# shanmo/OrcVIO

Measured on AMD Instinct MI355X. Metric: EKF updates/sec, 30 clones x 400 feats, higher is better.
Workload: dtype f64

## Files before the change

orcvio_amd/csrc/capi_handle.inc:

```

static double reg_lower_gamma(double a, double x) {
    if (x <= 0.0) return 0.0;
    const double lg = std::lgamma(a);
    if (x < a + 1.0) {
        double term = 1.0 / a, sum = term, ap = a;
        for (int i = 0; i < 200000; ++i) {
            ap += 1.0;
            term *= x / ap;
            sum += term;
            if (std::fabs(term) < std::fabs(sum) * 1e-17) break;
        }
        return sum * std::exp(a * std::log(x) - x - lg);
    }
    const double tiny = 1e-300;
    double b = x + 1.0 - a, c = 1.0 / tiny, d = 1.0 / b, h = d;
    for (int i = 1; i < 200000; ++i) {
        const double an = -(double)i * ((double)i - a);
        b += 2.0;
        d = an * d + b;
        if (std::fabs(d) < tiny) d = tiny;
        c = b + an / c;
        if (std::fabs(c) < tiny) c = tiny;
        d = 1.0 / d;
        const double del = d * c;
// ... 134 lines not shown
    size_t o = 0;
    for (int i = 0; i < n; ++i) {
        if (c[i].bytes == 0 || !c[i].dst) continue;
        HIPCHK(hipMemcpyAsync(h->h_fetch + o, c[i].src, c[i].bytes, hipMemcpyDeviceToHost, s));
        o += (c[i].bytes + 63) & ~(size_t)63;
    }
    HIPCHK(hipStreamSynchronize(s));
    o = 0;
    for (int i = 0; i < n; ++i) {
        if (c[i].bytes == 0 || !c[i].dst) continue;
        std::memcpy(c[i].dst, h->h_fetch + o, c[i].bytes);
        o += (c[i].bytes + 63) & ~(size_t)63;
    }
    return ORCVIO_OK;
}

static int launch_ingest(orcvio_msckf_handle* h, hipStream_t s, const void* src_dev, void* dst, size_t bytes, bool kernel = true,
                         int* zero = nullptr, unsigned zero_mask = 0u) {
    if (bytes == 0) return ORCVIO_OK;
    if (!kernel) {
        HIPCHK(hipMemcpyAsync(dst, src_dev, bytes, hipMemcpyHostToDevice, s));
        if (zero)
            for (int i = 0; i < 32; ++i)
                if (zero_mask >> i & 1u) HIPCHK(hipMemsetAsync(zero + i, 0, sizeof(int), s));
        return ORCVIO_OK;
    }
    const size_t n16 = (bytes + 15) / 16;
    int grid = (int)((n16 + 255) / 256);
    if (grid > 4 * h->n_cus) grid = 4 * h->n_cus;
    if (grid < 1) grid = 1;
    hipLaunchKernelGGL(k_ingest, dim3(grid), dim3(256), 0, s, reinterpret_cast<const u32x4*>(src_dev), reinterpret_cast<u32x4*>(dst), n16, zero, zero_mask);
    HIPCHK(hipGetLastError());
    return ORCVIO_OK;
}
static bool obj_ingest_kernel() {
    static const bool v = [] { const char* e = dbg_getenv("ORCVIO_OBJ_INGEST"); return e ? atoi(e) != 0 : true; }();
    return v;
}
static bool obj_publish_kernel() {
    static const bool v = [] { const char* e = dbg_getenv("ORCVIO_OBJ_PUBLISH"); return e ? atoi(e) != 0 : false; }();
    return v;
}
static void free_all(orcvio_msckf_handle* h) {
    (void)hipDeviceSynchronize();
    void* ptrs[] = {h->d_in, h->d_outs,
                    h->d_chi2, h->d_Hs, h->d_Gpart, h->d_Ab, h->d_A, h->d_RP,
                    h->d_DinvP, h->d_U, h->d_M, h->d_RM, h->d_DinvM, h->d_Z, h->d_La, h->d_DinvA,
                    h->d_W, h->d_Y, h->d_KG, h->d_Gobj, h->d_RF, h->d_DinvF, h->d_Yobj, h->d_objH,
                    h->d_obj_gamma, h->d_obj_i, h->d_obj_accept, h->d_T3, h->d_Xobs, h->d_S,
                    h->d_Pres, h->d_Ptmp, h->d_Sres, h->d_Stmp, h->d_covT, h->d_covmap, h->d_skip, h->d_tri_valid, h->d_tri_flags, h->d_tri_init, h->d_tri_sol, h->d_tri_cost, h->d_sync, h->d_la_rdy, h->d_U2, h->d_M2, h->d_RM2, h->d_DinvM2, h->d_Z2, h->d_outs2, h->d_chain_words, h->d_obj_done,
                    h->d_ekf_i, h->d_ekf_d, h->d_ekf_E, h->d_Gekf, h->d_ekf_gamma, h->d_ekf_accept, h->d_slam, h->d_dense, h->d_Rf, h->d_new, h->d_aug, h->d_split};
    for (void* p : ptrs)
        if (p) (void)hipFree(p);
    if (h->h_stage) (void)hipHostFree(h->h_stage);
    if (h->h_obj_stage) (void)hipHostFree(h->h_obj_stage);
    if (h->h_lm) (void)hipHostFree(h->h_lm);
    if (h->d_lm) (void)hipFree(h->d_lm);
    if (h->h_stage2) (void)hipHostFree(h->h_stage2);
    if (h->h_tri) (void)hipHostFree(h->h_tri);
    if (h->d_tri_words) (void)hipFree(h->d_tri_words);
    if (h->d_in2) (void)hipFree(h->d_in2);
    if (h->d_step_words) (void)hipFree(h->d_step_words);
    if (h->h_evt) (void)hipHostFree(h->h_evt);
    if (h->d_evt) (void)hipFree(h->d_evt);
    for (double* q : {h->d_Hthin, h->d_Vthin, h->d_uthin}) if (q) (void)hipFree(q);
    if (h->d_obj_in) (void)hipFree(h->d_obj_in);
// ... 338 lines not shown
```

orcvio_amd/csrc/capi_io.inc:

```

static int compute_optional(orcvio_msckf_handle* h, bool want_thin_or_K, bool want_K, bool want_G) {
    if (h->last_update_thin) { g_last_error = "H_thin / K / G are derived from the square-root path's factors: not available behind an update that took the direct form of a thin stack (ask for them in the update call itself)"; return ORCVIO_ERR_INVALID; }
    const int NA = h->NA, NAP = h->NAP, n = h->n, kf = h->kf - h->tail, NP = h->NP, ldz = h->ldz;
    hipStream_t s = h->stream;
    const PriorFactor pf = prior_factor(h);
    const long sLi = pf.sLi, sLj = pf.sLj;
    const double* La_P = pf.base + 15 * sLi;
    { const int ra = assemble_deferred(h, s); if (ra != ORCVIO_OK) return ra; }
    if (want_thin_or_K) {
        HIPCHK(hipMemcpyAsync(h->d_La, h->d_A, sizeof(double) * (size_t)NAP * NAP, hipMemcpyDeviceToDevice, s));
        hipLaunchKernelGGL(k_potrf, dim3(1), dim3(1024), 0, s, h->d_La, NA + 1, NAP, 0.0, h->d_DinvA, h->d_info + 4, 1e-11);
        HIPCHK(hipGetLastError());
    }
    if (want_G) {
        int rc = launch_trsm(h, s, h->d_RM, h->d_DinvM, kf, h->d_U, 1, NP, NA, nullptr, 0, h->d_W, NP);
        if (rc == ORCVIO_OK) rc = launch_gemm(s, h->d_Z, 1, ldz, h->d_W, NP, 1, n, NA, kf, 1.0, 0.0, 0, h->d_KG, NP, 1);
        if (rc != ORCVIO_OK) return rc;
    }
    if (want_K) {
        int rc = launch_gemm(s, La_P, sLj, sLi, h->d_La, NAP, 1, kf, NA, NA, 1.0, 0.0, 0, h->d_Y, NP, 1);
        if (rc == ORCVIO_OK) rc = launch_trsm(h, s, h->d_RM, h->d_DinvM, kf, h->d_Y, NP, 1, NA, nullptr, 0, h->d_W, NP);
        if (rc == ORCVIO_OK) rc = launch_gemm(s, h->d_Z, 1, ldz, h->d_W, NP, 1, n, NA, kf, 1.0, 0.0, 0, h->d_Y, NP, 1);
        if (rc != ORCVIO_OK) return rc;
    }
    HIPCHK(hipStreamSynchronize(s));
    return ORCVIO_OK;
}

static int download_enqueue(orcvio_msckf_handle* h, hipStream_t sd, bool with_P) {
    const size_t bytes = with_P ? h->oo_Pout + sizeof(double) * (size_t)h->n * h->n : h->outs_small;
    HIPCHK(hipMemcpyAsync(h->h_stage + h->in_cap + h->out_shift, h->d_outs, bytes, hipMemcpyDeviceToHost, sd));
    h->dl_pending = true; h->dl_with_P = with_P; h->dl_stream = sd;
    return ORCVIO_OK;
}

static int rerun_forked(orcvio_msckf_handle* h, hipStream_t s, bool want_P) {
    UpdateCall c;
    c.retry_forked = true;
    int rr = run_update_impl(h, s, c);
    if (rr == ORCVIO_OK) rr = download_enqueue(h, s ? s : h->stream, want_P);
    return rr;
}

static int download_impl(orcvio_msckf_handle* h, orcvio_msckf_result* res, bool retried) {
    if (!h || !res || !h->ran) { g_last_error = "download: no finished update"; return ORCVIO_ERR_INVALID; }
    HIPCHK(hipSetDevice(h->device));
    const int n = h->n, NA = h->NA, NAP = h->NAP, NP = h->NP, F = h->F;
    const bool want_P = res->P_out != nullptr;
    if (!(h->dl_pending && (h->dl_with_P || !want_P))) {
        hipStream_t sd = h->last_stream ? h->last_stream : h->stream;
        if (h->dl_pending) HIPCHK(hipStreamSynchronize(h->dl_stream));
        HIPCHK(hipStreamSynchronize(h->side));
        const int rq = download_enqueue(h, sd, want_P);
        if (rq != ORCVIO_OK) return rq;
    }
    HIPCHK(hipStreamSynchronize(h->dl_stream));
    h->dl_pending = false;
    if (h->last_sharded) {
        const int rl = ipc_check_lost(h, "orcvio_msckf_download");
        if (rl != ORCVIO_OK) return rl;
    }
    const char* so = h->h_stage + h->in_cap;
    const double* dx = reinterpret_cast<const double*>(so + h->oo_dx);
    const double* gam = reinterpret_cast<const double*>(so + h->oo_gamma);
    const int* acc = reinterpret_cast<const int*>(so + h->oo_accept);
    if (res->dx) std::memcpy(res->dx, dx, sizeof(double) * n);
    if (res->P_out) std::memcpy(res->P_out, so + h->oo_Pout, sizeof(double) * (size_t)n * n);
    if (res->accept && F > 0) std::memcpy(res->accept, acc, sizeof(int) * F);
    if (res->gamma && F > 0) std::memcpy(res->gamma, gam, sizeof(double) * F);
    int info[16] = {0};
    std::memcpy(info, so, sizeof(int) * 16);
// ... 40 lines not shown
        if (res->G) {
            std::vector<double> Gd((size_t)n * NP);
            HIPCHK(hipMemcpy(Gd.data(), h->d_KG, sizeof(double) * Gd.size(), hipMemcpyDeviceToHost));
            std::memset(res->G, 0, sizeof(double) * (size_t)n * n);
            for (int i = 0; i < n; ++i)
                for (int c = 0; c < NA; ++c) res->G[(size_t)i * n + 15 + c] = Gd[(size_t)i * NP + c];
        }
        if (res->K) {
            std::vector<double> Kd((size_t)n * NP);
            HIPCHK(hipMemcpy(Kd.data(), h->d_Y, sizeof(double) * Kd.size(), hipMemcpyDeviceToHost));
            for (int i = 0; i < n; ++i)
                for (int c = 0; c < NA; ++c) res->K[(size_t)i * NA + c] = Kd[(size_t)i * NP + c];
        }
    }
    return ORCVIO_OK;
}
int32_t orcvio_msckf_download(orcvio_msckf_handle* h, orcvio_msckf_result* res) { return download_impl(h, res, false); }

static int launch_triangulate(orcvio_msckf_handle* h, const orcvio_triangulation_config* cfg, bool have_init, bool mark_skip, hipStream_t s,
                              bool io, bool with_mode);
static inline void tri_consume(orcvio_msckf_handle* h, UpdateCall& c) {
    if (!h->tri_armed) return;
    h->tri_armed = false;
    c.tri = true;
    h->skip_active = true; h->tri_live = true;
    h->tri_refuse_empty = h->F > 0 && h->ekf_F == 0 && h->dense_rows == 0 && h->new_F == 0 && !c.info_also;
    if (h->tri_refuse_empty) c.info_also = h->d_tri_words;
}
static unsigned long long io_signature(const orcvio_msckf_handle* h, hipStream_t s, bool want_P, bool commit, const UpdateCall& c, bool finpub = false) {
    unsigned long long sig = launch_signature(h, s, h->h_stage_dev, (long)(0x100 | (want_P ? 1 : 0) | (commit ? 2 : 0) | (finpub ? 4 : 0)), c);
    auto mix = [&](unsigned long long v) { sig = (sig ^ v) * 1099511628211ull; };
    mix((unsigned long long)upload_bytes(h)); mix((unsigned long long)h->io_poses); mix((unsigned long long)(size_t)h->d_Stmp); mix((unsigned long long)(size_t)h->d_Pres);
    mix(h->factor_opt); mix((unsigned long long)h->outs_small); mix((unsigned long long)(size_t)h->d_Ptmp); mix(h->finpub_opt);
    mix(c.tri); mix(h->tri_live);
    if (c.tri) {
        const orcvio_triangulation_config& t = h->tri_cfg;
        const double d[6] = {t.translation_threshold, t.huber_epsilon, t.estimation_precision, t.initial_damping, t.cost_threshold, t.init_final_dist_threshold};
        for (double v : d) { unsigned long long bits; std::memcpy(&bits, &v, 8); mix(bits); }
        mix((unsigned long long)t.outer_loop_max_iteration); mix((unsigned long long)t.inner_loop_max_iteration);
        mix(h->tri_with_mode); mix((unsigned long long)(size_t)h->h_tri_dev); mix((unsigned long long)(size_t)c.info_also);
    }
    return sig;
}

static int step_words(orcvio_msckf_handle* h) {
    if (h->d_step_words) return ORCVIO_OK;
    HIPCHK(hipMalloc(&h->d_step_words, 256));
    HIPCHK(hipMemset(h->d_step_words, 0, 256));
    return ORCVIO_OK;
}

static inline bool finpub_active(const orcvio_msckf_handle* h, const UpdateCall& c) {
    return h->finpub_opt && !h->objects_mode && h->n_nui == 0 && !finish_fused_active(h, c);
}
static int io_enqueue(orcvio_msckf_handle* h, hipStream_t s, bool want_P, bool commit, UpdateCall& c, bool allow_finpub = false) {
    const int mode = commit ? (h->factor_opt && h->n_nui == 0 ? 2 : 1) : 0;
    const SolveOut so = solve_out(h);
    c.fin_pub = allow_finpub && finpub_active(h, c) && !want_P;
    if (c.fin_pub) c.pub = finish_pub_args(h, so, mode, c.info_also);
    h->last_finpub_commit = c.fin_pub && commit;
    int rc = ORCVIO_OK;
    if (!c.already_ingested) rc = launch_ingest(h, s, h->h_stage_dev, h->d_in, early_ingest() || (h->tri_live && !c.tri) ? h->io_poses : upload_bytes(h));
    if (rc == ORCVIO_OK && c.tri) rc = launch_triangulate(h, &h->tri_cfg, false, true, s, true, h->tri_with_mode);
    if (rc == ORCVIO_OK) rc = enqueue_update(h, s, c);
    if (rc != ORCVIO_OK || c.fin_pub) return rc;
    return launch_epilogue(s, epilogue_args(h, so, 0, want_P, mode, nullptr, c.info_also, c.info_keep));
}

static int io_wait(orcvio_msckf_handle* h, hipStream_t s, unsigned long long expected_pub) {
    const unsigned long long expected = expected_pub ? expected_pub : h->pub_enqueued;
    const auto t0 = std::chrono::steady_clock::now();
    unsigned spins = 0;
    bool late = false;
    while (__atomic_load_n(h->h_flag, __ATOMIC_ACQUIRE) < expected) {
        _mm_pause();
        if ((++spins & 4095u) == 0 &&
            std::chrono::duration<double>(std::chrono::steady_clock::now() - t0).count() > h->io_spin_seconds) { late = true; break; }
    }
    if (late) {
        HIPCHK(hipStreamSynchronize(s));
        const unsigned long long now = __atomic_load_n(h->h_flag, __ATOMIC_ACQUIRE);
        if (now < expected) {
            h->pub_enqueued = now;
            g_last_error = "io_update: the results were not published";
            return ORCVIO_ERR_TIMEOUT;
        }
    }
    return ORCVIO_OK;
}

struct FeatureView { int n, F, NA; size_t oo_dx, oo_gamma, oo_accept; const int* row_ptr; int discard_large_update; };
static inline FeatureView feature_view(const orcvio_msckf_handle* h) {
    return FeatureView{h->n, h->F, h->NA, h->oo_dx, h->oo_gamma, h->oo_accept, h->h_row_ptr.data(), h->flags.discard_large_update};
}
static int feature_outcome_view(orcvio_msckf_handle* h, const FeatureView& v, const char* so, int32_t* stats);
// ... 103 lines not shown
    return ORCVIO_OK;
}

int32_t orcvio_msckf_io_begin(orcvio_msckf_handle* h, const orcvio_msckf_flags* flags, int32_t n_clones, int32_t n_features,
                              int32_t n_observations, int32_t with_P, orcvio_msckf_io* io) {
    if (!h || !flags || !io) { g_last_error = "io_begin: null argument"; return ORCVIO_ERR_INVALID; }
    if (with_P < 0 || with_P > 2) { g_last_error = "io_begin: with_P is 0, 1 or 2"; return ORCVIO_ERR_INVALID; }
    const int rc = upload_begin(h, flags, n_clones, n_features, n_observations, with_P == 1, true, "orcvio_msckf_io_begin", with_P == 2);
    if (rc != ORCVIO_OK) return rc;
    char* st = h->h_stage;
    io->n = h->n;
    io->poses = reinterpret_cast<double*>(st + h->io_poses);
    io->obs_ptr = reinterpret_cast<int32_t*>(st + h->io_optr);
    io->p_w = reinterpret_cast<double*>(st + h->io_pw);
    io->obs_clone = reinterpret_cast<int32_t*>(st + h->io_oclone);
    io->obs_z = reinterpret_cast<double*>(st + h->io_z);
    io->obs_zvel = h->io_zvel != h->io_z ? reinterpret_cast<double*>(st + h->io_zvel) : nullptr;
    io->P = with_P == 1 ? reinterpret_cast<double*>(st + h->io_P) : nullptr;
    const char* so = st + h->in_cap;
    io->dx = reinterpret_cast<const double*>(so + h->oo_dx);
    io->gamma = reinterpret_cast<const double*>(so + h->oo_gamma);
    io->accept = reinterpret_cast<const int32_t*>(so + h->oo_accept);
    io->P_out = reinterpret_cast<const double*>(so + h->oo_Pout);
    h->io_open = true;
    return ORCVIO_OK;
}

int32_t orcvio_msckf_io_update(orcvio_msckf_handle* h, int32_t want_P, int32_t commit, int32_t* stats) {
    if (!h || !h->io_open) { g_last_error = "io_update: call orcvio_msckf_io_begin first"; return ORCVIO_ERR_INVALID; }
    if (h->io_submitted) { g_last_error = "io_update: an update submitted with orcvio_msckf_io_submit has not been collected"; return ORCVIO_ERR_INVALID; }
    static const bool timing = dbg_getenv("ORCVIO_TIMING") != nullptr;
    const auto tf0 = std::chrono::steady_clock::now();
    HIPCHK(hipSetDevice(h->device));
    int rc = ingest_raw(h, h->stream);
    if (rc != ORCVIO_OK) return rc;
    const auto tf1 = std::chrono::steady_clock::now();
    rc = upload_finalize(h, "orcvio_msckf_io_update");
    if (timing) {
        static int calls = 0;
        if ((++calls % 64) == 0)
            fprintf(stderr, "io_update: set device %.1f us, finalize %.1f us\n", std::chrono::duration<double, std::micro>(tf1 - tf0).count(),
                    std::chrono::duration<double, std::micro>(std::chrono::steady_clock::now() - tf1).count());
    }
    if (rc != ORCVIO_OK) {
        (void)arena_mark_read(h, h->stream);
        return rc;
    }
    h->pw_missing = false;
    h->io_open = true;
    UpdateCall c;
    tri_consume(h, c);
    return io_run(h, want_P != 0, commit != 0, stats, c);
}

int32_t orcvio_msckf_io_submit(orcvio_msckf_handle* h, int32_t want_P, int32_t commit) {
    if (!h || !h->io_open) { g_last_error = "io_submit: call orcvio_msckf_io_begin first"; return ORCVIO_ERR_INVALID; }
    if (h->io_submitted) { g_last_error = "io_submit: the previous submission has not been collected"; return ORCVIO_ERR_INVALID; }
    HIPCHK(hipSetDevice(h->device));
    int rc = ingest_raw(h, h->stream);
    if (rc == ORCVIO_OK) rc = upload_finalize(h, "orcvio_msckf_io_submit");
    if (rc != ORCVIO_OK) { (void)arena_mark_read(h, h->stream); return rc; }
    h->pw_missing = false;
    h->io_open = true;
    UpdateCall c;
    tri_consume(h, c);
    rc = io_launch(h, want_P != 0, commit != 0, c);
    if (rc != ORCVIO_OK) return rc;
    h->io_submitted = true; h->io_sub_P = want_P != 0; h->io_sub_commit = commit != 0;
    return ORCVIO_OK;
}
int32_t orcvio_msckf_io_collect(orcvio_msckf_handle* h, int32_t* stats) {
    if (!h || !h->io_submitted) { g_last_error = "io_collect: nothing submitted"; return ORCVIO_ERR_INVALID; }
    HIPCHK(hipSetDevice(h->device));
    h->io_submitted = false;
    return io_finish(h, h->io_sub_P, h->io_sub_commit, stats);
}

int32_t orcvio_msckf_update_features(orcvio_msckf_handle* h, const orcvio_msckf_flags* flags, const orcvio_msckf_window* window,
                                     const orcvio_msckf_tracks* tracks, const double* P, orcvio_msckf_result* result) {
    static const bool timing = dbg_getenv("ORCVIO_TIMING") != nullptr;
    if (!result) { g_last_error = "update_features: null result"; return ORCVIO_ERR_INVALID; }
    const auto t0 = std::chrono::steady_clock::now();
    int rc = upload_to_arena(h, flags, window, tracks, P, "orcvio_msckf_update_features", true);
    if (rc != ORCVIO_OK) return rc;
    const auto t1 = std::chrono::steady_clock::now();
    const bool want_P = result->P_out != nullptr;
    UpdateCall c;
    c.thin_blocked = result->H_thin || result->r_thin || result->K || result->G;
    rc = io_run(h, want_P, false, result->stats, c);
    const auto t3 = std::chrono::steady_clock::now();
    if (rc != ORCVIO_OK) return rc;
    const int n = h->n, F = h->F;
    const char* so = h->h_stage + h->in_cap;
    if (result->dx) std::memcpy(result->dx, so + h->oo_dx, sizeof(double) * n);
    if (result->P_out) std::memcpy(result->P_out, so + h->oo_Pout, sizeof(double) * (size_t)n * n);
    if (result->accept && F > 0) std::memcpy(result->accept, so + h->oo_accept, sizeof(int) * F);
    if (result->gamma && F > 0) std::memcpy(result->gamma, so + h->oo_gamma, sizeof(double) * F);
    if (result->H_thin || result->r_thin || result->K || result->G) {
        orcvio_msckf_result opt = *result;
        opt.dx = nullptr; opt.P_out = nullptr; opt.accept = nullptr; opt.gamma = nullptr;
        rc = orcvio_msckf_download(h, &opt);
        if (rc != ORCVIO_OK) return rc;
    }
    const auto t4 = std::chrono::steady_clock::now();
    if (timing) {
        auto us = [](auto a, auto b) { return std::chrono::duration<double, std::micro>(b - a).count(); };
        static int calls = 0;
        if (us(t0, t4) > 2000.0 || (++calls % 64) == 0)
            fprintf(stderr, "update_features: staging %.0f us, launch + wait %.0f us, unpack %.0f us\n", us(t0, t1), us(t1, t3), us(t3, t4));
    }
    return rc;
}

int32_t orcvio_msckf_gate_tracks(orcvio_msckf_handle* h, const orcvio_msckf_flags* flags, const orcvio_msckf_window* window,
                                 const orcvio_msckf_tracks* tracks, const double* P, double* gamma, int32_t* accept) {
    if (!gamma || !accept) { g_last_error = "gate_tracks: null output"; return ORCVIO_ERR_INVALID; }
    int rc = orcvio_msckf_upload(h, flags, window, tracks, P);
    if (rc != ORCVIO_OK) return rc;
    if (h->pw_missing) { g_last_error = "gate_tracks: tracks without positions"; return ORCVIO_ERR_INVALID; }
    const int F = h->F;
// ... 11 lines not shown
```

orcvio_amd/csrc/capi_update.inc:

```

static int upload_begin(orcvio_msckf_handle* h, const orcvio_msckf_flags* flags, int N, int F, int nobs, bool with_P, bool have_zvel,
                        const char* who, bool pending_aug = false) {
    if (flags->leg_dim != 22 && flags->leg_dim != 46) { g_last_error = std::string(who) + ": leg_dim must be 22 or 46"; return ORCVIO_ERR_INVALID; }
    if (N < 1 || F < 0) { g_last_error = std::string(who) + ": bad sizes"; return ORCVIO_ERR_INVALID; }
    if (h->io_submitted) { g_last_error = std::string(who) + ": an update submitted with orcvio_msckf_io_submit has not been collected"; return ORCVIO_ERR_INVALID; }
    HIPCHK(hipSetDevice(h->device));
    { const int rw = arena_wait_free(h); if (rw != ORCVIO_OK) return rw; }
    if (h->dl_pending) { HIPCHK(hipStreamSynchronize(h->dl_stream)); h->dl_pending = false; }
    if (N > h->maxN || F > h->maxF) { g_last_error = std::string(who) + ": exceeds handle capacity"; return ORCVIO_ERR_CAPACITY; }
    if (nobs < 0) { g_last_error = std::string(who) + ": obs_ptr not monotone"; return ORCVIO_ERR_INVALID; }
    if (nobs > h->maxObs) { g_last_error = std::string(who) + ": too many observations"; return ORCVIO_ERR_CAPACITY; }
    if (flags->estimate_td && F > 0 && !have_zvel) { g_last_error = std::string(who) + ": obs_zvel required with estimate_td"; return ORCVIO_ERR_INVALID; }
    const int n = flags->leg_dim + 6 * N + h->n_extra;
    if (n > h->n_max) { g_last_error = "window + extra states exceed the handle's capacity"; return ORCVIO_ERR_CAPACITY; }
    if (6 * h->n_nui > h->n_extra || N + h->n_nui > h->maxN) { g_last_error = std::string(who) + ": nuisance states do not fit the extra states / the pose capacity"; return ORCVIO_ERR_CAPACITY; }
    if (!with_P && h->res_n != n && !(pending_aug && n <= h->res_n + 6)) { g_last_error = std::string(who) + ": P == NULL but the resident covariance does not match the window"; return ORCVIO_ERR_INVALID; }
    h->uploaded = false; h->ran = false; h->io_open = false;
    h->tri_armed = false;
    h->last_update_thin = false;
    h->flags = *flags;
    h->N = N; h->F = F; h->nobs = nobs;
    h->n = n;
    h->NA = h->ekf_mode ? h->n - 15 : flags->leg_dim + 6 * N - 15;
    h->ekf_F = 0; h->dense_rows = 0; h->new_F = 0;
    h->NAP = round_up(h->NA + 1, 16);
    if (h->chi2_prob_cached != flags->chi2_prob) {
        h->h_chi2.assign(ORCVIO_CHI2_TABLE, 0.0);
        for (int d = 1; d < ORCVIO_CHI2_TABLE; ++d) h->h_chi2[d] = orcvio_msckf_chi2_quantile(d, flags->chi2_prob);
        HIPCHK(hipMemcpyAsync(h->d_chi2, h->h_chi2.data(), sizeof(double) * ORCVIO_CHI2_TABLE, hipMemcpyHostToDevice, h->stream));
        HIPCHK(hipStreamSynchronize(h->stream));
        h->chi2_prob_cached = flags->chi2_prob;
    }
    const bool with_zvel = have_zvel && flags->estimate_td;
    layout_inputs(h, N + h->n_nui, F, nobs, with_zvel, with_P, h->n);
    layout_outputs(h, h->n, F);
    h->io_with_P = with_P;
    return ORCVIO_OK;
}

static inline size_t upload_bytes(const orcvio_msckf_handle* h) {
    return h->io_with_P ? h->io_P + sizeof(double) * (size_t)h->n * h->n : h->in_used;
}
static bool early_ingest() {
    static const bool v = [] { const char* e = dbg_getenv("ORCVIO_EARLY_INGEST"); return e ? atoi(e) != 0 : true; }();
    return v;
}
static int ingest_raw(orcvio_msckf_handle* h, hipStream_t s) {
    if (!early_ingest()) return ORCVIO_OK;
    return launch_ingest(h, s, h->h_stage_dev + h->io_poses, h->d_in + h->io_poses, upload_bytes(h) - h->io_poses);
}

static int upload_finalize(orcvio_msckf_handle* h, const char* who) {
    const int N = h->N, F = h->F, nobs = h->nobs;
    if (!h->io_with_P) {
        if (h->res_n != h->n) { g_last_error = std::string(who) + ": P == NULL but the resident covariance does not match the window"; return ORCVIO_ERR_INVALID; }
        h->d_P = h->d_Pres;
    }
    select_prior_factor(h, h->io_with_P);
    h->NP = round_up(h->n > h->kf ? h->n : h->kf, 16);
    h->ldz = round_up(h->n + 1, 16);
    h->reg_path = (h->NP / 16) <= 14;
    select_tail(h);
    { const int rcl = factor_layout_clean(h); if (rcl != ORCVIO_OK) return rcl; }
    char* st = h->h_stage;
    const int* obs_ptr = reinterpret_cast<const int*>(st + h->io_optr);
    const int* obs_clone = reinterpret_cast<const int*>(st + h->io_oclone);
    if (F > 0 && obs_ptr[0] < 0) { g_last_error = std::string(who) + ": obs_ptr starts below zero"; return ORCVIO_ERR_INVALID; }
    if (F > 0 && obs_ptr[F] != nobs) { g_last_error = std::string(who) + ": obs_ptr[F] differs from the number of observations"; return ORCVIO_ERR_INVALID; }
    h->h_row_ptr.resize(F + 1);
    int* row_ptr = h->h_row_ptr.data();
    row_ptr[0] = 0;
    int Mmax = 2;
    for (int j = 0; j < F; ++j) {
        const int M = obs_ptr[j + 1] - obs_ptr[j];
        if (M < 0) { g_last_error = std::string(who) + ": obs_ptr not monotone"; return ORCVIO_ERR_INVALID; }
        if (M > ORCVIO_MAX_TRACK) { g_last_error = std::string(who) + ": track longer than ORCVIO_MAX_TRACK"; return ORCVIO_ERR_TRACK_TOO_LONG; }
        if (M > Mmax) Mmax = M;
        row_ptr[j + 1] = row_ptr[j] + (M >= 2 ? 2 * M - 3 : 0);
    }
    std::memcpy(st + h->io_rptr, row_ptr, sizeof(int) * (F + 1));
    {
        int cnt[ORCVIO_MAX_CLONES + 2] = {0};
        unsigned bad = 0;
        std::vector<unsigned char>& is_run = h->track_is_run;
        is_run.resize(F > 0 ? F : 1);
        const int o_first = F > 0 ? obs_ptr[0] : 0;
        for (int j = 0; j < F; ++j) {
            const int o0 = obs_ptr[j], M = obs_ptr[j + 1] - o0;
            const int* oc = obs_clone + o0;
            const int c0 = M > 0 ? oc[0] : 0;
            unsigned brk = 0;
            for (int k = 0; k < M; ++k) brk |= (unsigned)(oc[k] != c0 + k);
            const bool run = !brk && c0 >= 0 && c0 + M <= N;
            is_run[j] = run;
            if (run) {
                int* cc = cnt + c0 + 1;
// ... 3 lines not shown
                    const unsigned c = (unsigned)oc[k];
                    bad |= (c >= (unsigned)N);
                    cnt[(c < (unsigned)N ? c : 0u) + 1]++;
                }
            }
        }
        for (int o = 0; o < o_first; ++o) {
            const unsigned c = (unsigned)obs_clone[o];
            bad |= (c >= (unsigned)N);
            cnt[(c < (unsigned)N ? c : 0u) + 1]++;
        }
        if (bad) { g_last_error = std::string(who) + ": obs_clone out of range"; return ORCVIO_ERR_INVALID; }
        for (int i = 0; i < N; ++i) cnt[i + 1] += cnt[i];
        int* clone_obs = reinterpret_cast<int*>(st + h->io_cobs);
        int fill[ORCVIO_MAX_CLONES + 2];
        std::memcpy(fill, cnt, sizeof(int) * (N + 1));
        for (int o = 0; o < o_first; ++o) clone_obs[o] = fill[obs_clone[o]]++;
        for (int j = 0; j < F; ++j) {
            const int o0 = obs_ptr[j], M = obs_ptr[j + 1] - o0;
            if (M <= 0) continue;
            if (is_run[j]) {
                int* __restrict__ out = clone_obs + o0;
                int* __restrict__ ff = fill + obs_clone[o0];
                for (int k = 0; k < M; ++k) out[k] = ff[k];
                for (int k = 0; k < M; ++k) ff[k] += 1;
            } else {
                for (int k = 0; k < M; ++k) clone_obs[o0 + k] = fill[obs_clone[o0 + k]]++;
            }
        }
        int* cptr = reinterpret_cast<int*>(st + h->io_cptr);
        for (int i = 0; i <= N; ++i) cptr[i] = 2 * cnt[i];
        h->s_chunks = N;
    }
    h->m_tot = row_ptr[F];
    h->Mmax = Mmax;
    int chunks = (3 * F + 1023) / 1024;
    if (chunks > h->gram_chunks_cap) chunks = h->gram_chunks_cap;
    if (chunks < 1) chunks = 1;
    const int t3rows = 3 * F;
    int rpc = round_up((t3rows + chunks - 1) / chunks, 8);
    if (rpc < 8) rpc = 8;
    h->rows_per_chunk = rpc;
    h->chunks = t3rows > 0 ? (t3rows + rpc - 1) / rpc : 1;
    h->uploaded = true;
    h->ran = false;
    h->skip_active = false; h->tri_live = false; h->tri_refuse_empty = false;
    h->objects_mode = false;
    return feature_split_reserve(h);
}

static void stage_inputs(orcvio_msckf_handle* h, const orcvio_msckf_window* w, const orcvio_msckf_tracks* tr, const double* P) {
    const int N = h->N, F = h->F, nobs = h->nobs;
    char* st = h->h_stage;
    if (P) std::memcpy(st + h->io_P, P, sizeof(double) * (size_t)h->n * h->n);
    double* poses = reinterpret_cast<double*>(st + h->io_poses);
    const double* tfej = w->t_fej ? w->t_fej : w->t_b_w;
    for (int i = 0; i < N; ++i) {
        double* r = poses + (size_t)POSE_STRIDE * i;
        std::memcpy(r + POSE_R_B2W, w->R_b2w + 9 * i, 9 * sizeof(double));
        std::memcpy(r + POSE_T_B_W, w->t_b_w + 3 * i, 3 * sizeof(double));
        std::memcpy(r + POSE_T_FEJ, tfej + 3 * i, 3 * sizeof(double));
        std::memcpy(r + POSE_R_B2C, w->R_b2c + 9 * i, 9 * sizeof(double));
        std::memcpy(r + POSE_T_C_B, w->t_c_b + 3 * i, 3 * sizeof(double));
        r[27] = 0.0;
    }
    std::memcpy(st + h->io_optr, tr->obs_ptr, sizeof(int) * (F + 1));
    if (F > 0) {
        if (tr->p_w) std::memcpy(st + h->io_pw, tr->p_w, sizeof(double) * 3 * F);
        else std::memset(st + h->io_pw, 0, sizeof(double) * 3 * F);
        if (nobs > 0) {
            std::memcpy(st + h->io_oclone, tr->obs_clone, sizeof(int) * nobs);
            std::memcpy(st + h->io_z, tr->obs_z, sizeof(double) * 2 * nobs);
            if (h->io_zvel != h->io_z) std::memcpy(st + h->io_zvel, tr->obs_zvel, sizeof(double) * 2 * nobs);
        }
    }
}

static int upload_to_arena(orcvio_msckf_handle* h, const orcvio_msckf_flags* flags, const orcvio_msckf_window* w,
                           const orcvio_msckf_tracks* tr, const double* P, const char* who, bool early_ingest = false) {
    if (!h || !flags || !w || !tr || !w->R_b2w || !w->t_b_w || !w->R_b2c || !w->t_c_b || !tr->obs_ptr) {
        g_last_error = std::string(who) + ": null argument";
        return ORCVIO_ERR_INVALID;
    }
    const int N = w->n_clones, F = tr->n_features;
    if (N < 1 || F < 0) { g_last_error = std::string(who) + ": bad sizes"; return ORCVIO_ERR_INVALID; }
    if (F > h->maxF) { g_last_error = std::string(who) + ": exceeds handle capacity"; return ORCVIO_ERR_CAPACITY; }
    if (F > 0 && tr->obs_ptr[0] < 0) { g_last_error = std::string(who) + ": obs_ptr starts below zero"; return ORCVIO_ERR_INVALID; }
    const int nobs = F > 0 ? tr->obs_ptr[F] : 0;
    if (F > 0 && nobs > 0 && (!tr->obs_clone || !tr->obs_z)) { g_last_error = std::string(who) + ": null track arrays"; return ORCVIO_ERR_INVALID; }
    int rc = upload_begin(h, flags, N, F, nobs, P != nullptr, tr->obs_zvel != nullptr, who);
    if (rc != ORCVIO_OK) return rc;
    stage_inputs(h, w, tr, P);
    if (early_ingest) { rc = ingest_raw(h, h->stream); if (rc != ORCVIO_OK) return rc; }
    rc = upload_finalize(h, who);
    if (rc != ORCVIO_OK) return rc;
    h->pw_missing = (F > 0 && !tr->p_w);
    return ORCVIO_OK;
}

int32_t orcvio_msckf_upload(orcvio_msckf_handle* h, const orcvio_msckf_flags* flags, const orcvio_msckf_window* w,
                            const orcvio_msckf_tracks* tr, const double* P) {
    const int rc = upload_to_arena(h, flags, w, tr, P, "orcvio_msckf_upload");
    if (rc != ORCVIO_OK) return rc;
    HIPCHK(hipMemcpyAsync(h->d_in, h->h_stage, upload_bytes(h), hipMemcpyHostToDevice, h->stream));
    return arena_mark_read(h, h->stream);
}

static FeatArgs feature_args(const orcvio_msckf_handle* h) {
    FeatArgs a;
    a.poses = h->d_poses; a.p_w = h->d_pw; a.obs_ptr = h->d_obs_ptr; a.obs_clone = h->d_obs_clone;
    a.obs_z = h->d_obs_z; a.obs_zvel = h->d_obs_zvel; a.P = h->d_P; a.row_ptr = h->d_row_ptr; a.chi2 = h->d_chi2;
    a.skip = h->skip_active ? h->d_skip : nullptr;
    a.Hs = h->materialize ? h->d_Hs : nullptr; a.T3 = h->d_T3; a.Xobs = h->d_Xobs; a.obs_pos = h->d_clone_obs; a.gamma = h->d_gamma; a.accept = h->d_accept; a.Rf = h->d_Rf;
    a.sigma2 = h->flags.noise_feature * h->flags.noise_feature;
    a.n = h->n; a.leg = h->flags.leg_dim; a.N = h->N; a.NA = h->NA; a.NAP = h->NAP; a.Mmax = h->Mmax; a.F = h->F;
    a.use_larvio = h->flags.use_larvio; a.use_left = h->flags.use_left_perturbation; a.if_fej = h->flags.if_fej;
    a.estimate_td = h->flags.estimate_td;
    a.ablate = h->feat_ablate;
    return a;
}

static bool feature_split_active(const orcvio_msckf_handle* h) {
    return h->split_min_tracks > 0 && h->F >= h->split_min_tracks && !h->materialize && h->feat_ablate == 0 && (h->NAP + 63) / 64 <= 7 &&
           feat_split_lds_bytes(h->Mmax, h->NAP, h->N) <= (size_t)40 * 1024;
}
static int feature_split_reserve(orcvio_msckf_handle* h) {
    if (!feature_split_active(h)) return ORCVIO_OK;
    const size_t need = (size_t)h->F * feat_split_track_doubles(h->Mmax);
// ... 733 lines not shown
```

orcvio_amd/csrc/io_ops.hpp:

```cpp
#pragma once
#include <hip/hip_runtime.h>

namespace orcvio_amd {

typedef unsigned int u32x4 __attribute__((ext_vector_type(4)));

__global__ __launch_bounds__(256) void k_ingest(const u32x4* __restrict__ src, u32x4* __restrict__ dst, size_t n16, int* __restrict__ zero = nullptr,
                                                unsigned zero_mask = 0u) {
    if (zero && blockIdx.x == 0 && threadIdx.x < 32 && (zero_mask >> threadIdx.x & 1u)) zero[threadIdx.x] = 0;
    const size_t stride = (size_t)gridDim.x * 256;
    for (size_t i = (size_t)blockIdx.x * 256 + threadIdx.x; i < n16; i += stride) dst[i] = __builtin_nontemporal_load(src + i);
}

struct EpilogueArgs {
    const u32x4* small_src; u32x4* small_dst; size_t small16;
    const u32x4* P_src; u32x4* P_dst; size_t P16; int nb_P;
    int commit;
    const double* Pout; double* Pres; size_t nn;
    const double* Z; int ldz, kf, n; double sigma;
    const double* prior; long sLi, sLj; double* Sout; int ldo;
    const double* dx; const int* info;
    const int* accept;
    int* counter;
    unsigned long long* seq;
    unsigned long long* flag;
    const int* info_also;
    int* info_keep;
    int pub_all;
};
__global__ __launch_bounds__(256) void k_epilogue(EpilogueArgs a) {
    const int nb = gridDim.x, b = blockIdx.x, t = threadIdx.x;
    if (b == 0) {
        if (a.info_keep && t < 16) a.info_keep[t] = a.info[t];
        for (size_t i = t; i < a.small16; i += 256) a.small_dst[i] = a.small_src[i];
    } else if (b <= a.nb_P) {
        const size_t stride = (size_t)a.nb_P * 256;
        for (size_t i = (size_t)(b - 1) * 256 + t; i < a.P16; i += stride) a.P_dst[i] = a.P_src[i];
    } else if (a.commit) {
        __shared__ int s_bad;
        if (t == 0) s_bad = 0;
        __syncthreads();
        int bad = 0;
        for (int i = t; i < a.n; i += 256) { const double v = a.dx[i]; bad |= !(v - v == 0.0); }
        if (bad) s_bad = 1;
// ... 69 lines not shown
```

orcvio_amd/csrc/msckf_capi.hip:

```cpp
#include "../../include/orcvio_msckf.h"

#include <hip/hip_runtime.h>
#include <rccl/rccl.h>
#include <dlfcn.h>
#include <chrono>

#include <algorithm>
#include <array>
#include <cmath>
#include <cstdio>
#include <cstring>
#include <string>
#include <vector>

#include <functional>
#include "msckf_kernels.hpp"
#include "feature_split.hpp"
#include "triangulate.hpp"
#include "triangulate_arm.hpp"
#include "cov_ops.hpp"
#include "zupt_ops.hpp"
#include "ekf_rows.hpp"
#include "object_rows.hpp"
#include "object_fused.hpp"
// ... 49 lines not shown
    orcvio_msckf_flags flags{};
    int N = 0, F = 0, nobs = 0, n = 0, NA = 0, NAP = 0, NP = 0, ldz = 0, m_tot = 0, Mmax = 0;
    int chunks = 0, rows_per_chunk = 0;
    bool uploaded = false, ran = false;
    bool reg_path = true;
    bool fused_solve = true;
    int* d_skip = nullptr;
    bool skip_active = false;
    char *d_in = nullptr, *d_outs = nullptr;
    char* h_stage = nullptr;
    size_t in_cap = 0, outs_cap = 0, in_used = 0, outs_small = 0, stage_bytes = 0;
    size_t io_poses = 0, io_optr = 0, io_rptr = 0, io_cptr = 0, io_pw = 0, io_oclone = 0, io_cobs = 0, io_z = 0, io_zvel = 0, io_P = 0;
    size_t oo_dx = 0, oo_gamma = 0, oo_accept = 0, oo_Pout = 0;
    bool dl_pending = false, dl_with_P = false;
    hipStream_t dl_stream = nullptr;
    static constexpr int GRAPH_WAYS = 6;
    struct GraphSlot {
        struct Way { hipGraph_t graph = nullptr; hipGraphExec_t exec = nullptr; unsigned long long sig = 0, used = 0; };
        Way way[GRAPH_WAYS];
        unsigned long long seen[8] = {0, 0, 0, 0, 0, 0, 0, 0};
        int seen_at = 0;
        unsigned long long tick = 0;
    };
    GraphSlot g_update, g_local, g_finish, g_io;
    char* h_stage_dev = nullptr;
    unsigned long long* h_flag = nullptr;
    unsigned long long* h_flag_dev = nullptr;
    unsigned long long* d_seq = nullptr;
    int* d_pubcnt = nullptr;
    unsigned long long pub_enqueued = 0;
    bool io_submitted = false, io_sub_P = false, io_sub_commit = false;
    bool io_open = false, io_with_P = false;
    double io_spin_seconds = 2.0;
    bool last_sharded = false;
    hipEvent_t* shard_ev = nullptr;
    int ranks_seen = 0;
    int shard_status = 0;
    hipStream_t last_stream = nullptr;
    double *d_Pres = nullptr, *d_Ptmp = nullptr, *d_covT = nullptr;
    double *d_Sres = nullptr, *d_Stmp = nullptr;
    int fac_n = 0, fac_k = 0, fac_ld = 0;
    bool fac_valid = false;
    bool factor_opt = true;
    int n_nui = 0;
    bool obj_dof_rank = false;
    bool ref_h2_ldlt = false;
    bool ref_stack_hf = false;
    int obj_refine_mode = 1;
    int obj_refined = 0;
    size_t obj_fused_budget = 0;
    int obj_fused_opt = 1;
    unsigned* d_obj_done = nullptr;
    unsigned obj_done_total = 0u;
    int early_rows_tot = 0, early_no_max = 0, early_dof = 0, early_Fmax = 1; size_t early_nd = 0, early_ni = 0;
    bool obj_early_done = false;
    bool obj_last_fused = false;
    size_t obj_lds_budget = 0;
    bool arrow_opt = true;
    bool use_factor = false;
    bool rev_prior_opt = true;
    int tail = 0, fac_tail = 0;
    hipStream_t obj_stream = nullptr;
    hipEvent_t ev_obj = nullptr;
    bool frame_mode = false;
    size_t out_shift = 0;
    char* h_fetch = nullptr;
// ... 117 lines not shown
    int gram_chunks_cap = 64;
    std::vector<double> h_poses, h_chi2;
    std::vector<int> h_row_ptr;
    std::vector<unsigned char> track_is_run;
    std::vector<int> frame_row_ptr;
    char *d_in2 = nullptr, *h_stage2 = nullptr, *h_stage2_dev = nullptr;
    bool arena_swapped = false;
    char *h_evt = nullptr, *h_evt_dev = nullptr, *d_evt = nullptr;
    int* d_step_words = nullptr;
    std::vector<int> step_row_ptr;
    long long cnt_step_frames = 0, cnt_step_repairs = 0;
    bool ekf_one_launch = true;
    bool finpub_opt = true;
    bool last_finpub_commit = false;
    bool thin_opt = true;
    double *d_Hthin = nullptr, *d_Vthin = nullptr, *d_uthin = nullptr;
    bool last_update_thin = false;
    bool step_fused = true;
    bool ekf_side_opt = true;
    bool ekf_side_used = false;
    long long ekf_side_skip_until = 0;
    unsigned ekf_side_seq = 0;
    double chi2_prob_cached = -1.0;
};

struct UpdateCall {
    bool fin_pub = false;
    FinishPubArgs pub{};
    int* info_keep = nullptr;
    const int* info_also = nullptr;
    bool fin_frame = false;
    bool ekf_side = false;
    bool already_ingested = false;
    bool tri = false;
    unsigned* mark_M_word = nullptr;
    unsigned mark_M_val = 0u;
    const unsigned* join_wait = nullptr;
    unsigned join_expect = 0u;
    bool thin_blocked = false;
    bool retry_forked = false;
    const std::function<int()>* mid = nullptr;
    unsigned* front_mark = nullptr; unsigned front_mark_val = 0;
    const unsigned* asm_wait = nullptr; unsigned asm_wait_val = 0;
    bool front_did_U = false;
};

struct CovState { double *Pres, *Ptmp, *Sres, *Stmp; int res_n, fac_n, fac_k, fac_ld, fac_tail; bool fac_valid; };
static inline CovState cov_state(const orcvio_msckf_handle* h) {
    return CovState{h->d_Pres, h->d_Ptmp, h->d_Sres, h->d_Stmp, h->res_n, h->fac_n, h->fac_k, h->fac_ld, h->fac_tail, h->fac_valid};
}
static inline void cov_restore(orcvio_msckf_handle* h, const CovState& c) {
    h->d_Pres = c.Pres; h->d_Ptmp = c.Ptmp; h->d_Sres = c.Sres; h->d_Stmp = c.Stmp;
    h->res_n = c.res_n; h->fac_n = c.fac_n; h->fac_k = c.fac_k; h->fac_ld = c.fac_ld; h->fac_tail = c.fac_tail; h->fac_valid = c.fac_valid;
}
static inline void fac_adopt(orcvio_msckf_handle* h, int n, int k, int ld, int tail) {
    std::swap(h->d_Sres, h->d_Stmp);
    h->fac_n = n; h->fac_k = k; h->fac_ld = ld; h->fac_tail = tail; h->fac_valid = true;
}
static inline void fac_adopt_update(orcvio_msckf_handle* h) {
    fac_adopt(h, h->n, h->kf, h->ldz, h->tail);
    h->res_n = h->n;
}
static inline void commit_bookkeeping(orcvio_msckf_handle* h) {
    if (h->last_finpub_commit) { std::swap(h->d_Pres, h->d_Ptmp); h->last_finpub_commit = false; }
    if (h->last_update_thin) h->fac_valid = false;
    else if (h->factor_opt && h->n_nui == 0) fac_adopt(h, h->n, h->kf, h->ldz, h->tail);
// ... 39 lines not shown
```

Measured before the change: 7749.

## Fuse raw and header ingest into one flag-gated pull kernel

Replaces the two separate ingest launches (raw payload early, pose/header region later) with a single k_pull kernel. Some blocks copy the linear payload right away, while others spin on a host-written sequence flag and copy the header region once the host finishes finalizing it. The host releases the flag midway through upload_finalize, so the header copy overlaps the remaining CPU work and one kernel launch is saved per update. In exchange it adds a GPU spin-wait with a timeout and a cancel path, new state tracking (pull_carried, derived_pulled), and a fallback re-ingest for forked retries.

```diff
diff --git a/orcvio_amd/csrc/capi_handle.inc b/orcvio_amd/csrc/capi_handle.inc
--- a/orcvio_amd/csrc/capi_handle.inc
+++ b/orcvio_amd/csrc/capi_handle.inc
@@ -190,6 +190,38 @@
     hipLaunchKernelGGL(k_ingest, dim3(grid), dim3(256), 0, s, reinterpret_cast<const u32x4*>(src_dev), reinterpret_cast<u32x4*>(dst), n16, zero, zero_mask);
     HIPCHK(hipGetLastError());
     return ORCVIO_OK;
+}
+static double pull_wait_seconds() {
+    static const double v = [] { const char* e = dbg_getenv("ORCVIO_PULL_WAIT_S"); const double s = e ? atof(e) : 0.0; return s > 0.0 ? s : 2.0; }();
+    return v;
+}
+static int launch_pull(orcvio_msckf_handle* h, hipStream_t s, size_t lin_bytes) {
+    PullArgs a{};
+    a.lin_src = reinterpret_cast<const u32x4*>(h->h_stage_dev + h->io_poses);
+    a.lin_dst = reinterpret_cast<u32x4*>(h->d_in + h->io_poses);
+    a.lin16 = (lin_bytes + 15) / 16;
+    a.nlin = (int)((a.lin16 + 255) / 256);
+    if (a.nlin > 4 * h->n_cus) a.nlin = 4 * h->n_cus;
+    a.head_src = reinterpret_cast<const u32x4*>(h->h_stage_dev);
+    a.head_dst = reinterpret_cast<u32x4*>(h->d_in);
+    a.head16 = h->io_poses / 16;
+    a.nhead = (int)((a.head16 + 255) / 256);
+    if (a.nhead > 64) a.nhead = 64;
+    if (a.nhead < 1) a.nhead = 1;
+    a.word = h->h_flag_dev + 16;
+    a.ticks = (unsigned long long)(pull_wait_seconds() * 1e8);
+    a.lost = h->d_info + 8;
+    a.seq = ++h->pull_seq;
+    h->pull_live = true;
+    const int grid = a.nlin + a.nhead;
+    hipLaunchKernelGGL(k_pull, dim3(grid), dim3(256), 0, s, a);
+    HIPCHK(hipGetLastError());
+    return ORCVIO_OK;
+}
+static inline void pull_release(orcvio_msckf_handle* h, bool cancelled) {
+    if (!h->pull_live) return;
+    h->pull_live = false;
+    __atomic_store_n(h->h_flag + 16, h->pull_seq | (cancelled ? ORCVIO_PULL_CANCELLED : 0ull), __ATOMIC_RELEASE);
 }
 static bool obj_ingest_kernel() {
     static const bool v = [] { const char* e = dbg_getenv("ORCVIO_OBJ_INGEST"); return e ? atoi(e) != 0 : true; }();
diff --git a/orcvio_amd/csrc/capi_io.inc b/orcvio_amd/csrc/capi_io.inc
--- a/orcvio_amd/csrc/capi_io.inc
+++ b/orcvio_amd/csrc/capi_io.inc
@@ -37,6 +37,7 @@
 static int rerun_forked(orcvio_msckf_handle* h, hipStream_t s, bool want_P) {
     UpdateCall c;
     c.retry_forked = true;
+    if (h->pull_carried) { const int ri = launch_ingest(h, s ? s : h->stream, h->h_stage_dev, h->d_in, h->io_poses); if (ri != ORCVIO_OK) return ri; }
     int rr = run_update_impl(h, s, c);
     if (rr == ORCVIO_OK) rr = download_enqueue(h, s ? s : h->stream, want_P);
     return rr;
@@ -143,7 +144,7 @@
     auto mix = [&](unsigned long long v) { sig = (sig ^ v) * 1099511628211ull; };
     mix((unsigned long long)upload_bytes(h)); mix((unsigned long long)h->io_poses); mix((unsigned long long)(size_t)h->d_Stmp); mix((unsigned long long)(size_t)h->d_Pres);
     mix(h->factor_opt); mix((unsigned long long)h->outs_small); mix((unsigned long long)(size_t)h->d_Ptmp); mix(h->finpub_opt);
-    mix(c.tri); mix(h->tri_live);
+    mix(c.tri); mix(h->tri_live); mix(c.derived_pulled);
     if (c.tri) {
         const orcvio_triangulation_config& t = h->tri_cfg;
         const double d[6] = {t.translation_threshold, t.huber_epsilon, t.estimation_precision, t.initial_damping, t.cost_threshold, t.init_final_dist_threshold};
@@ -171,7 +172,7 @@
     if (c.fin_pub) c.pub = finish_pub_args(h, so, mode, c.info_also);
     h->last_finpub_commit = c.fin_pub && commit;
     int rc = ORCVIO_OK;
-    if (!c.already_ingested) rc = launch_ingest(h, s, h->h_stage_dev, h->d_in, early_ingest() || (h->tri_live && !c.tri) ? h->io_poses : upload_bytes(h));
+    if (!c.already_ingested && !c.derived_pulled) rc = launch_ingest(h, s, h->h_stage_dev, h->d_in, early_ingest() || (h->tri_live && !c.tri) ? h->io_poses : upload_bytes(h));
     if (rc == ORCVIO_OK && c.tri) rc = launch_triangulate(h, &h->tri_cfg, false, true, s, true, h->tri_with_mode);
     if (rc == ORCVIO_OK) rc = enqueue_update(h, s, c);
     if (rc != ORCVIO_OK || c.fin_pub) return rc;
@@ -341,7 +342,7 @@
     static const bool timing = dbg_getenv("ORCVIO_TIMING") != nullptr;
     const auto tf0 = std::chrono::steady_clock::now();
     HIPCHK(hipSetDevice(h->device));
-    int rc = ingest_raw(h, h->stream);
+    int rc = ingest_raw(h, h->stream, true);
     if (rc != ORCVIO_OK) return rc;
     const auto tf1 = std::chrono::steady_clock::now();
     rc = upload_finalize(h, "orcvio_msckf_io_update");
@@ -358,6 +359,7 @@
     h->pw_missing = false;
     h->io_open = true;
     UpdateCall c;
+    c.derived_pulled = h->pull_carried;
     tri_consume(h, c);
     return io_run(h, want_P != 0, commit != 0, stats, c);
 }
@@ -366,12 +368,13 @@
     if (!h || !h->io_open) { g_last_error = "io_submit: call orcvio_msckf_io_begin first"; return ORCVIO_ERR_INVALID; }
     if (h->io_submitted) { g_last_error = "io_submit: the previous submission has not been collected"; return ORCVIO_ERR_INVALID; }
     HIPCHK(hipSetDevice(h->device));
-    int rc = ingest_raw(h, h->stream);
+    int rc = ingest_raw(h, h->stream, true);
     if (rc == ORCVIO_OK) rc = upload_finalize(h, "orcvio_msckf_io_submit");
     if (rc != ORCVIO_OK) { (void)arena_mark_read(h, h->stream); return rc; }
     h->pw_missing = false;
     h->io_open = true;
     UpdateCall c;
+    c.derived_pulled = h->pull_carried;
     tri_consume(h, c);
     rc = io_launch(h, want_P != 0, commit != 0, c);
     if (rc != ORCVIO_OK) return rc;
@@ -395,6 +398,7 @@
     const auto t1 = std::chrono::steady_clock::now();
     const bool want_P = result->P_out != nullptr;
     UpdateCall c;
+    c.derived_pulled = h->pull_carried;
     c.thin_blocked = result->H_thin || result->r_thin || result->K || result->G;
     rc = io_run(h, want_P, false, result->stats, c);
     const auto t3 = std::chrono::steady_clock::now();
diff --git a/orcvio_amd/csrc/capi_update.inc b/orcvio_amd/csrc/capi_update.inc
--- a/orcvio_amd/csrc/capi_update.inc
+++ b/orcvio_amd/csrc/capi_update.inc
@@ -16,6 +16,7 @@
     if (6 * h->n_nui > h->n_extra || N + h->n_nui > h->maxN) { g_last_error = std::string(who) + ": nuisance states do not fit the extra states / the pose capacity"; return ORCVIO_ERR_CAPACITY; }
     if (!with_P && h->res_n != n && !(pending_aug && n <= h->res_n + 6)) { g_last_error = std::string(who) + ": P == NULL but the resident covariance does not match the window"; return ORCVIO_ERR_INVALID; }
     h->uploaded = false; h->ran = false; h->io_open = false;
+    h->pull_carried = false;
     h->tri_armed = false;
     h->last_update_thin = false;
     h->flags = *flags;
@@ -45,12 +46,28 @@
     static const bool v = [] { const char* e = dbg_getenv("ORCVIO_EARLY_INGEST"); return e ? atoi(e) != 0 : true; }();
     return v;
 }
-static int ingest_raw(orcvio_msckf_handle* h, hipStream_t s) {
+static bool pull_one() {
+    static const bool v = [] { const char* e = dbg_getenv("ORCVIO_PULL_ONE"); return e ? atoi(e) != 0 : true; }();
+    return v;
+}
+static int ingest_raw(orcvio_msckf_handle* h, hipStream_t s, bool carry = false) {
+    h->pull_carried = false;
     if (!early_ingest()) return ORCVIO_OK;
-    return launch_ingest(h, s, h->h_stage_dev + h->io_poses, h->d_in + h->io_poses, upload_bytes(h) - h->io_poses);
-}
-
+    if (!carry || !pull_one())
+        return launch_ingest(h, s, h->h_stage_dev + h->io_poses, h->d_in + h->io_poses, upload_bytes(h) - h->io_poses);
+    const int rc = launch_pull(h, s, upload_bytes(h) - h->io_poses);
+    if (rc != ORCVIO_OK) { pull_release(h, true); return rc; }
+    h->pull_carried = true;
+    return ORCVIO_OK;
+}
+
+static int upload_finalize_arena(orcvio_msckf_handle* h, const char* who);
 static int upload_finalize(orcvio_msckf_handle* h, const char* who) {
+    const int rc = upload_finalize_arena(h, who);
+    pull_release(h, true);
+    return rc;
+}
+static int upload_finalize_arena(orcvio_msckf_handle* h, const char* who) {
     const int N = h->N, F = h->F, nobs = h->nobs;
     if (!h->io_with_P) {
         if (h->res_n != h->n) { g_last_error = std::string(who) + ": P == NULL but the resident covariance does not match the window"; return ORCVIO_ERR_INVALID; }
@@ -61,7 +78,6 @@
     h->ldz = round_up(h->n + 1, 16);
     h->reg_path = (h->NP / 16) <= 14;
     select_tail(h);
-    { const int rcl = factor_layout_clean(h); if (rcl != ORCVIO_OK) return rcl; }
     char* st = h->h_stage;
     const int* obs_ptr = reinterpret_cast<const int*>(st + h->io_optr);
     const int* obs_clone = reinterpret_cast<const int*>(st + h->io_oclone);
@@ -131,6 +147,8 @@
         for (int i = 0; i <= N; ++i) cptr[i] = 2 * cnt[i];
         h->s_chunks = N;
     }
+    pull_release(h, false);
+    { const int rcl = factor_layout_clean(h); if (rcl != ORCVIO_OK) return rcl; }
     h->m_tot = row_ptr[F];
     h->Mmax = Mmax;
     int chunks = (3 * F + 1023) / 1024;
@@ -190,9 +208,12 @@
     int rc = upload_begin(h, flags, N, F, nobs, P != nullptr, tr->obs_zvel != nullptr, who);
     if (rc != ORCVIO_OK) return rc;
     stage_inputs(h, w, tr, P);
-    if (early_ingest) { rc = ingest_raw(h, h->stream); if (rc != ORCVIO_OK) return rc; }
+    if (early_ingest) { rc = ingest_raw(h, h->stream, true); if (rc != ORCVIO_OK) return rc; }
     rc = upload_finalize(h, who);
-    if (rc != ORCVIO_OK) return rc;
+    if (rc != ORCVIO_OK) {
+        if (early_ingest) (void)arena_mark_read(h, h->stream);
+        return rc;
+    }
     h->pw_missing = (F > 0 && !tr->p_w);
     return ORCVIO_OK;
 }
diff --git a/orcvio_amd/csrc/io_ops.hpp b/orcvio_amd/csrc/io_ops.hpp
--- a/orcvio_amd/csrc/io_ops.hpp
+++ b/orcvio_amd/csrc/io_ops.hpp
@@ -10,6 +10,45 @@
     if (zero && blockIdx.x == 0 && threadIdx.x < 32 && (zero_mask >> threadIdx.x & 1u)) zero[threadIdx.x] = 0;
     const size_t stride = (size_t)gridDim.x * 256;
     for (size_t i = (size_t)blockIdx.x * 256 + threadIdx.x; i < n16; i += stride) dst[i] = __builtin_nontemporal_load(src + i);
+}
+
+#define ORCVIO_PULL_CANCELLED (1ull << 63)
+struct PullArgs {
+    const u32x4* lin_src; u32x4* lin_dst; size_t lin16; int nlin;
+    const u32x4* head_src; u32x4* head_dst; size_t head16; int nhead;
+    const unsigned long long* word; unsigned long long seq, ticks; int* lost;
+};
+__global__ __launch_bounds__(256) void k_pull(PullArgs a) {
+    const int b = blockIdx.x, t = threadIdx.x;
+    if (b < a.nlin) {
+        const size_t stride = (size_t)a.nlin * 256;
+        for (size_t i = (size_t)b * 256 + t; i < a.lin16; i += stride) a.lin_dst[i] = __builtin_nontemporal_load(a.lin_src + i);
+        return;
+    }
+    __shared__ int s_go;
+    if (t == 0) {
+        int go = 1;
+        const unsigned long long t0 = wall_clock64();
+        for (;;) {
+            const unsigned long long w = __hip_atomic_load(a.word, __ATOMIC_ACQUIRE, __HIP_MEMORY_SCOPE_SYSTEM);
+            if (w == a.seq) break;
+            if ((w & ~ORCVIO_PULL_CANCELLED) >= a.seq) { go = 0; break; }
+            if (wall_clock64() - t0 > a.ticks) { go = -1; break; }
+            __builtin_amdgcn_s_sleep(8);
+        }
+        s_go = go;
+    }
+    __syncthreads();
+    const int go = s_go;
+    if (go == 0) return;
+    const size_t stride = (size_t)a.nhead * 256, first = (size_t)(b - a.nlin) * 256 + t;
+    if (go < 0) {
+        for (size_t i = first; i < a.head16; i += stride) a.head_dst[i] = u32x4{0u, 0u, 0u, 0u};
+        if (t == 0) atomicAdd(a.lost, 1);
+        return;
+    }
+    __builtin_amdgcn_fence(__ATOMIC_ACQUIRE, "");
+    for (size_t i = first; i < a.head16; i += stride) a.head_dst[i] = __builtin_nontemporal_load(a.head_src + i);
 }
 
 struct EpilogueArgs {
diff --git a/orcvio_amd/csrc/msckf_capi.hip b/orcvio_amd/csrc/msckf_capi.hip
--- a/orcvio_amd/csrc/msckf_capi.hip
+++ b/orcvio_amd/csrc/msckf_capi.hip
@@ -105,6 +105,9 @@
     bool io_submitted = false, io_sub_P = false, io_sub_commit = false;
     bool io_open = false, io_with_P = false;
     double io_spin_seconds = 2.0;
+    unsigned long long pull_seq = 0;
+    bool pull_live = false;
+    bool pull_carried = false;
     bool last_sharded = false;
     hipEvent_t* shard_ev = nullptr;
     int ranks_seen = 0;
@@ -288,6 +291,7 @@
     bool fin_frame = false;
     bool ekf_side = false;
     bool already_ingested = false;
+    bool derived_pulled = false;
     bool tri = false;
     unsigned* mark_M_word = nullptr;
     unsigned mark_M_val = 0u;
```

Result: no change. 7824 (median of 2 runs) (+1.0%).
